# rnaarla/advanced-rag-milvus

Measured on AMD Instinct MI355X. Metric: queries_per_sec_hybrid_retrieve, higher is better.
Workload: dtype f16

## Files before the change

### advanced-rag-milvus_amd/advanced_rag/_native.py

```python
from __future__ import annotations

import ctypes
import os
import threading
from typing import Optional, Sequence, Tuple

import numpy as np

from .staging import csr_of_queries

HR_F32, HR_F16 = 0, 1
HR_METRIC_IP, HR_METRIC_COSINE, HR_METRIC_L2 = 0, 1, 2
HR_METHOD_SEMANTIC, HR_METHOD_SPARSE, HR_METHOD_DOMAIN = 1, 2, 4
HR_MAX_TOPK = 256
HR_NORM_COSINE, HR_NORM_ATAN, HR_NORM_ATAN_DIST, HR_NORM_MINMAX, HR_NORM_MINMAX_DIST = 0, 1, 2, 3, 4
HR_DECAY_GAUSS, HR_DECAY_EXP, HR_DECAY_LINEAR = 0, 1, 2
HR_NORM_NONE = -1
HR_COL_F64 = 5
HR_MAX_DEEP_K = 16384
HR_N_PHASES = 10
PHASE_NAMES = ("prep", "dense_scan", "group_select", "refine", "topk",
               "sparse_scan", "sparse_select", "sparse_refine", "sparse_topk", "finish_fused")
HR_DEBUG_FINISH_MODE, HR_DEBUG_FAIL_NEXT_BUILD, HR_DEBUG_DENSE_KERNELS, HR_DEBUG_SPARSE_RPB, HR_DEBUG_GROUP_ROWS = 1, 2, 3, 4, 5
HR_DEBUG_NO_TRIM = 6
# ... 100 lines not shown
    "hr_decay_rerank_dev": (_c.c_int, [_c.c_void_p, _c.c_void_p, _c.c_int, _c.c_void_p, _c.c_int, _c.c_int, _c.c_void_p, _c.c_int,
                                       _c.c_int64, _c.c_int64, _c.c_void_p, _c.c_int, _c.c_int, _c.c_void_p, _c.c_void_p, _c.c_void_p,
                                       _c.c_void_p, _c.c_void_p]),
    "hr_mask_drop_groups_dev": (_c.c_int, [_c.c_void_p, _c.c_void_p, _c.c_int64, _c.c_void_p, _c.c_void_p, _c.c_int, _c.c_void_p]),
    "hr_group_select_n_dev": (_c.c_int, [_c.c_void_p, _c.c_void_p, _c.c_int, _c.c_int, _c.c_void_p, _c.c_int64, _c.c_int64, _c.c_int,
                                         _c.c_int, _c.c_void_p, _c.c_void_p, _c.c_void_p, _c.c_void_p, _c.c_void_p, _c.c_void_p]),
    "hr_mask_keep_groups_dev": (_c.c_int, [_c.c_void_p, _c.c_void_p, _c.c_int64, _c.c_void_p, _c.c_void_p, _c.c_int, _c.c_void_p]),
    "hr_add_layernorm_f16_dev": (_c.c_int, [_c.c_void_p, _c.c_void_p, _c.c_void_p, _c.c_void_p, _c.c_void_p, _c.c_int64,
                                            _c.c_int, _c.c_float, _c.c_void_p]),
    "hr_embed_layernorm_f16_dev": (_c.c_int, [_c.c_void_p, _c.c_void_p, _c.c_void_p, _c.c_void_p, _c.c_void_p, _c.c_void_p,
                                              _c.c_void_p, _c.c_void_p, _c.c_int64, _c.c_int, _c.c_int, _c.c_float, _c.c_int64,
                                              _c.c_int64, _c.c_void_p]),
    "hr_attention_f16_dev": (_c.c_int, [_c.c_void_p, _c.c_void_p, _c.c_void_p, _c.c_int64, _c.c_int, _c.c_int, _c.c_int,
                                        _c.c_float, _c.c_void_p]),
    "hr_attention_rows_f16_dev": (_c.c_int, [_c.c_void_p, _c.c_int64, _c.c_int64, _c.c_void_p, _c.c_void_p, _c.c_int64, _c.c_int64,
                                             _c.c_void_p, _c.c_void_p, _c.c_int64, _c.c_int, _c.c_int, _c.c_int, _c.c_int, _c.c_float,
                                             _c.c_void_p]),
    "hr_linear_rows_f16_dev": (_c.c_int, [_c.c_void_p, _c.c_int, _c.c_void_p, _c.c_void_p, _c.c_void_p, _c.c_int64, _c.c_int, _c.c_int,
                                          _c.c_int64, _c.c_void_p]),
    "hr_attention_fr_f16_dev": (_c.c_int, [_c.c_void_p, _c.c_void_p, _c.c_void_p, _c.c_int64, _c.c_int, _c.c_int, _c.c_int,
                                           _c.c_float, _c.c_void_p]),
    "hr_encoder_tail_f16_dev": (_c.c_int, [_c.c_void_p, _c.c_void_p, _c.c_int, _c.c_void_p, _c.c_int, _c.c_void_p, _c.c_void_p,
                                           _c.c_int64, _c.c_int, _c.c_int, _c.c_float, _c.c_int, _c.c_void_p]),
    "hr_mask_rows_scratch_bytes": (_c.c_size_t, [_c.c_int64]),
    "hr_mask_rows_dev": (_c.c_int, [_c.c_void_p, _c.c_int64, _c.c_int64, _c.c_int64, _c.c_int64, _c.c_void_p, _c.c_void_p,
                                    _c.c_void_p, _c.c_void_p]),
    "hr_get_dense_rows_dev": (_c.c_int, [_c.c_void_p, _c.c_void_p, _c.c_int64, _c.c_int, _c.c_void_p, _c.c_int64, _c.c_void_p,
                                         _c.c_void_p]),
    "hr_get_dense_rows": (_c.c_int, [_c.c_void_p, _c.c_void_p, _c.c_int64, _c.c_void_p]),
    "hr_get_sparse_rows_scratch_bytes": (_c.c_size_t, [_c.c_int64]),
    "hr_get_sparse_rows_dev": (_c.c_int, [_c.c_void_p, _c.c_void_p, _c.c_int64, _c.c_void_p, _c.c_void_p, _c.c_void_p, _c.c_int64,
                                          _c.c_void_p, _c.c_void_p, _c.c_void_p]),
    "hr_get_sparse_rows": (_c.c_int, [_c.c_void_p, _c.c_void_p, _c.c_int64, _c.c_void_p, _c.c_void_p, _c.c_void_p, _c.c_int64,
                                      _c.c_void_p]),
    "hr_search_dense_deep": (_c.c_int, [_c.c_void_p, _c.c_void_p, _c.c_int, _c.c_int, _c.c_int, _c.c_void_p, _c.c_int, _c.c_void_p,
                                        _c.c_void_p]),
    "hr_search_sparse_deep": (_c.c_int, [_c.c_void_p, _c.c_void_p, _c.c_void_p, _c.c_void_p, _c.c_int, _c.c_int, _c.c_int,
                                         _c.c_float, _c.c_void_p, _c.c_int, _c.c_void_p, _c.c_void_p]),
    "hr_deep_topk_scratch_bytes": (_c.c_size_t, [_c.c_int64, _c.c_int, _c.c_int]),
    "hr_deep_topk_dev": (_c.c_int, [_c.c_void_p, _c.c_void_p, _c.c_int64, _c.c_int, _c.c_int, _c.c_int, _c.c_int, _c.c_int64,
                                    _c.c_void_p, _c.c_void_p, _c.c_void_p, _c.c_void_p]),
    "hr_set_profiling": (_c.c_int, [_c.c_void_p, _c.c_int]),
    "hr_last_kernel_ms": (_c.c_int, [_c.c_void_p, _c.c_void_p, _c.c_int]),
    "hr_last_compact_ms": (_c.c_int, [_c.c_void_p, _c.c_void_p, _c.c_int]),
}
EXPORTED_SYMBOLS = tuple(_SIGNATURES)
# ... 666 lines not shown
    if rc != 0:
        _raise_global(L, rc)


def attention_fr_f16_dev(d_qkv: int, d_lengths: int, d_out_fr: int, n_seq: int, T: int, heads: int, head_dim: int, scale: float,
                         stream: int = 0):
    L = load_library()
    rc = L.hr_attention_fr_f16_dev(_vp(d_qkv), _vp(d_lengths) if d_lengths else None, _vp(d_out_fr), n_seq, T, heads, head_dim,
                                   float(scale), _vp(stream) if stream else None)
    if rc != 0:
        _raise_global(L, rc)


def encoder_tail_f16_dev(d_attn_fr: int, d_x: int, x_fr: bool, d_out: int, out_fr: bool, d_wstream: int, d_tables: int, rows: int,
                         hidden: int, intermediate: int, eps: float, gelu_erf: bool, stream: int = 0):
    L = load_library()
    rc = L.hr_encoder_tail_f16_dev(_vp(d_attn_fr), _vp(d_x), 1 if x_fr else 0, _vp(d_out), 1 if out_fr else 0, _vp(d_wstream),
                                   _vp(d_tables), rows, hidden, intermediate, float(eps), 1 if gelu_erf else 0,
                                   _vp(stream) if stream else None)
    if rc != 0:
        _raise_global(L, rc)


def attention_rows_f16_dev(d_q: int, q_seq_stride: int, q_token_stride: int, d_k: int, d_v: int, kv_seq_stride: int,
                           kv_token_stride: int, d_lengths: int, d_out: int, n_seq: int, T: int, n_queries: int, heads: int,
                           head_dim: int, scale: float, stream: int = 0):
    L = load_library()
    rc = L.hr_attention_rows_f16_dev(_vp(d_q), q_seq_stride, q_token_stride, _vp(d_k), _vp(d_v), kv_seq_stride, kv_token_stride,
                                     _vp(d_lengths) if d_lengths else None, _vp(d_out), n_seq, T, n_queries, heads, head_dim,
                                     float(scale), _vp(stream) if stream else None)
    if rc != 0:
        _raise_global(L, rc)


def rerank_linear_dev(d_ids: int, d_scores: int, d_methods: int, d_n: int, B: int, k_in: int, base_w: float,
                      method_bonus: float, recency_w: float, k_out: int, d_out_ids: int, d_out_scores: int,
                      d_out_orig: int, stream: int = 0, d_recency: int = 0):
    L = load_library()
    rc = L.hr_rerank_linear_dev(_vp(d_ids), _vp(d_scores), _vp(d_methods), _vp(d_n),
                                _vp(d_recency) if d_recency else None, B, k_in, base_w, method_bonus, recency_w,
                                k_out, _vp(d_out_ids), _vp(d_out_scores), _vp(d_out_orig),
                                _vp(stream) if stream else None)
    if rc != 0:
        _raise_global(L, rc)
```

### advanced-rag-milvus_amd/advanced_rag/encoder_kernels.py

```python
from __future__ import annotations

from typing import Optional

import torch

from . import _native

SUPPORTED_TAIL = {(384, 1536)}
SUPPORTED_LINEAR_K = {384}


def pack_natural(w: torch.Tensor) -> torch.Tensor:
    N, K = w.shape
    assert N % 16 == 0 and K % 32 == 0, (N, K)
    v = w.to(torch.float16).reshape(N // 16, 16, K // 32, 4, 8)
    return v.permute(0, 2, 3, 1, 4).contiguous().reshape(-1)


def pack_accumulator_order(w: torch.Tensor) -> torch.Tensor:
    N, K = w.shape
    assert N % 16 == 0 and K % 32 == 0, (N, K)
    v = w.to(torch.float16).reshape(N // 16, 16, K // 32, 2, 4, 4)
    return v.permute(0, 2, 4, 1, 3, 5).contiguous().reshape(-1)

# ... 10 lines not shown
    wp = w[perm]
    return (pack_accumulator_order(wp) if fragment_order_input else pack_natural(wp)), bias[perm].to(torch.float32).contiguous()


def pack_tail_stream(w_out: torch.Tensor, w_up: torch.Tensor, w_down: torch.Tensor) -> torch.Tensor:
    H, I = w_out.shape[0], w_up.shape[0]
    assert w_out.shape == (H, H) and w_up.shape == (I, H) and w_down.shape == (H, I) and H % 32 == 0 and I % 64 == 0
    piece = 512
    sp = H // 16
    out_p = pack_accumulator_order(w_out).reshape(-1, sp * piece)
    up_p = pack_accumulator_order(w_up).reshape(I // 32, sp * piece)
    down_p = pack_accumulator_order(w_down).reshape(H // 16, I // 32, piece).permute(1, 0, 2).reshape(I // 32, sp * piece)
    n = I // 32
    stages = [out_p, up_p[0:1]]
    inter = torch.stack([up_p[1:], down_p[:-1]], dim=1).reshape(2 * (n - 1), sp * piece)
    stages += [inter, down_p[-1:]]
    return torch.cat(stages).reshape(-1).contiguous()


def tail_tables(b_out, g1, be1, b_down, g2, be2, b_up) -> torch.Tensor:
    return torch.cat([t.reshape(-1).to(torch.float32) for t in (b_out, g1, be1, b_down, g2, be2, b_up)]).contiguous()


class LayerKernels:

    def __init__(self):
        self._key = None
        self.qkv_w = self.qkv_w_fr = self.qkv_b = self.kv_w = self.kv_w_fr = self.kv_b = self.stream = self.tables = None

    @staticmethod
    def supports(layer) -> bool:
        H, I = layer.out.weight.shape[0], layer.up.weight.shape[0]
        return (H, I) in SUPPORTED_TAIL and H in SUPPORTED_LINEAR_K

    def ensure(self, layer) -> "LayerKernels":
        params = (layer.qkv.weight, layer.qkv.bias, layer.out.weight, layer.out.bias, layer.ln1.weight, layer.ln1.bias,
                  layer.up.weight, layer.up.bias, layer.down.weight, layer.down.bias, layer.ln2.weight, layer.ln2.bias)
        key = tuple((p.data_ptr(), p._version) for p in params)
        if key != self._key:
            H = layer.out.weight.shape[0]
            with torch.no_grad():
                self.qkv_w, self.qkv_b = pack_linear(layer.qkv.weight, layer.qkv.bias, False)
                self.qkv_w_fr, _ = pack_linear(layer.qkv.weight, layer.qkv.bias, True)
                self.kv_w, self.kv_b = pack_linear(layer.qkv.weight[H:], layer.qkv.bias[H:], False)
                self.kv_w_fr, _ = pack_linear(layer.qkv.weight[H:], layer.qkv.bias[H:], True)
                self.stream = pack_tail_stream(layer.out.weight, layer.up.weight, layer.down.weight)
                self.tables = tail_tables(layer.out.bias, layer.ln1.weight, layer.ln1.bias, layer.down.bias,
                                          layer.ln2.weight, layer.ln2.bias, layer.up.bias)
            self._key = key
        return self


def fr_rows(rows: int) -> int:
    return -(-rows // 16) * 16


def to_fragment_order(x2d: torch.Tensor) -> torch.Tensor:
    M, H = x2d.shape
    pad = torch.zeros((fr_rows(M), H), dtype=x2d.dtype, device=x2d.device)
    pad[:M] = x2d
    v = pad.reshape(-1, 16, H // 32, 2, 4, 4)
    return v.permute(0, 2, 4, 1, 3, 5).contiguous().reshape(fr_rows(M), H)


def from_fragment_order(x_fr: torch.Tensor, rows: int) -> torch.Tensor:
    H = x_fr.shape[1]
    v = x_fr.reshape(-1, H // 32, 4, 16, 2, 4)
    return v.permute(0, 3, 1, 4, 2, 5).contiguous().reshape(-1, H)[:rows]


def linear_rows(x2d: torch.Tensor, w_packed: torch.Tensor, bias_f32: torch.Tensor, n_out: int, rows: Optional[int] = None,
                x_fr: bool = False, out: Optional[torch.Tensor] = None) -> torch.Tensor:
    M = x2d.shape[0] if rows is None else rows
    K = x2d.shape[1]
    if out is None:
        out = torch.empty((M, n_out), dtype=torch.float16, device=x2d.device)
    _native.linear_rows_f16_dev(x2d.data_ptr(), x_fr, w_packed.data_ptr(), bias_f32.data_ptr(), out.data_ptr(), M, K, n_out,
                                out.stride(0), torch.cuda.current_stream(x2d.device).cuda_stream)
    return out


def encoder_tail(attn_fr: torch.Tensor, x2d: torch.Tensor, k: LayerKernels, intermediate: int, eps: float, gelu_erf: bool,
                 rows: Optional[int] = None, x_fr: bool = False, out_fr: bool = False) -> torch.Tensor:
    M = x2d.shape[0] if rows is None else rows
    H = x2d.shape[1]
    out = torch.empty((fr_rows(M) if out_fr else M, H), dtype=torch.float16, device=x2d.device)
    _native.encoder_tail_f16_dev(attn_fr.data_ptr(), x2d.data_ptr(), x_fr, out.data_ptr(), out_fr, k.stream.data_ptr(),
                                 k.tables.data_ptr(), M, H, intermediate, eps, gelu_erf,
                                 torch.cuda.current_stream(x2d.device).cuda_stream)
    return out
```

### advanced-rag-milvus_amd/advanced_rag/encoders.py

```python
from __future__ import annotations

import math
import re
import zlib
from dataclasses import dataclass
from typing import Dict, List, Optional, Sequence, Tuple

import numpy as np
import torch
import torch.nn as nn
import torch.nn.functional as F

from . import _native
from .encoder_kernels import LayerKernels, encoder_tail, fr_rows, linear_rows

_WORD = re.compile(r"\w+|[^\w\s]")
PAD, CLS, SEP = 0, 101, 102


@dataclass
class EncoderConfig:
    vocab_size: int = 30522
    hidden: int = 384
    layers: int = 6
    heads: int = 12
    intermediate: int = 1536
    max_len: int = 512
    type_vocab: int = 2
    eps: float = 1e-12
    gelu: str = "tanh"


class HashTokenizer:

    _MEMO_MAX = 1 << 20

    def __init__(self, vocab_size: int = 30522, max_len: int = 512):
# ... 79 lines not shown

class _Layer(nn.Module):
    def __init__(self, c: EncoderConfig):
        super().__init__()
        self.heads = c.heads
        self.gelu = c.gelu
        self.qkv = nn.Linear(c.hidden, 3 * c.hidden)
        self.out = nn.Linear(c.hidden, c.hidden)
        self.ln1 = nn.LayerNorm(c.hidden, eps=c.eps)
        self.up = nn.Linear(c.hidden, c.intermediate)
        self.down = nn.Linear(c.intermediate, c.hidden)
        self.ln2 = nn.LayerNorm(c.hidden, eps=c.eps)
        self.kernels = LayerKernels()
        self.use_layer_kernels = True

    def _hip_attention_ok(self, x, lengths, hd, T) -> bool:
        return (lengths is not None and x.is_cuda and x.dtype == torch.float16 and
                ((hd == 32 and T <= 1024) or (hd == 64 and T <= 512)))

    def _fused_ok(self, x, lengths, hd, T) -> bool:
        return (self.use_layer_kernels and not getattr(_SMALL, "gemms", False) and self._hip_attention_ok(x, lengths, hd, T)
                and self.gelu in ("tanh", "erf") and LayerKernels.supports(self))

    def forward_fused(self, x2, B, T, lengths, x_fr: bool = False, out_fr: bool = False):
        H = x2.shape[1]
        hd = H // self.heads
        M = B * T
        k = self.kernels.ensure(self)
        if not x2.is_contiguous():
            x2 = x2.contiguous()
        qkv = linear_rows(x2, k.qkv_w_fr if x_fr else k.qkv_w, k.qkv_b, 3 * H, rows=M, x_fr=x_fr)
        a = torch.empty((fr_rows(M), H), dtype=x2.dtype, device=x2.device)
        _native.attention_fr_f16_dev(qkv.data_ptr(), lengths.data_ptr(), a.data_ptr(), B, T, self.heads, hd, hd ** -0.5,
                                     torch.cuda.current_stream(x2.device).cuda_stream)
        return encoder_tail(a, x2, k, self.up.weight.shape[0], float(self.ln1.eps), self.gelu == "erf", rows=M, x_fr=x_fr,
                            out_fr=out_fr)

    def forward(self, x, attn_bias, lengths=None):
        B, T, H = x.shape
        hd = H // self.heads
        if self._fused_ok(x, lengths, hd, T):
            return self.forward_fused(x.reshape(B * T, H), B, T, lengths).view(B, T, H)
        qkv = self.qkv(x)
        if self._hip_attention_ok(x, lengths, hd, T):
            qkv = qkv.contiguous()
            a = torch.empty((B, T, H), dtype=x.dtype, device=x.device)
            _native.attention_f16_dev(qkv.data_ptr(), lengths.data_ptr(), a.data_ptr(), B, T, self.heads, hd, hd ** -0.5,
                                      torch.cuda.current_stream(x.device).cuda_stream)
        else:
            q, k, v = qkv.view(B, T, 3, self.heads, hd).permute(2, 0, 3, 1, 4)
            a = F.scaled_dot_product_attention(q, k, v, attn_mask=attn_bias).transpose(1, 2).reshape(B, T, H)
        x = add_layer_norm(x, self.out(a), self.ln1)
        return add_layer_norm(x, self.down(self._ffn_up(x)), self.ln2)

    def forward_first_token(self, x, mask, lengths=None):
        B, T, H = x.shape
        hd = H // self.heads
        W, b = self.qkv.weight, self.qkv.bias
        if self._fused_ok(x, lengths, hd, T):
            k = self.kernels.ensure(self)
            x2 = x.reshape(B * T, H)
            kv = linear_rows(x2 if x2.is_contiguous() else x2.contiguous(), k.kv_w, k.kv_b, 2 * H).view(B, T, 2 * H)
        else:
            kv = F.linear(x, W[H:], b[H:])
        q = F.linear(x[:, 0], W[:H], b[:H])
        if self._hip_attention_ok(x, lengths, hd, T):
            kv, q = kv.contiguous(), q.contiguous()
            a = torch.empty((B, 1, H), dtype=x.dtype, device=x.device)
            _native.attention_rows_f16_dev(q.data_ptr(), H, 0, kv.data_ptr(), kv.data_ptr() + 2 * H, T * 2 * H, 2 * H,
                                           lengths.data_ptr(), a.data_ptr(), B, T, 1, self.heads, hd, hd ** -0.5,
                                           torch.cuda.current_stream(x.device).cuda_stream)
        else:
            kv = kv.view(B, T, 2, self.heads, hd)
            k, v = kv[:, :, 0].permute(0, 2, 1, 3), kv[:, :, 1].permute(0, 2, 1, 3)
            s = torch.matmul(q.view(B, self.heads, 1, hd), k.transpose(-1, -2)).float() * (hd ** -0.5)
            s = s.masked_fill(~mask[:, None, None, :], float("-inf"))
            a = torch.matmul(torch.softmax(s, dim=-1).to(x.dtype), v).reshape(B, 1, H)
        x0 = add_layer_norm(x[:, :1], self.out(a), self.ln1)
        return add_layer_norm(x0, self.down(self._ffn_up(x0)), self.ln2)

    def _ffn_up(self, x):
        if self.gelu != "tanh":
            return F.gelu(self.up(x))
        if x.is_cuda:
            B, T, H = x.shape
            return torch._addmm_activation(self.up.bias, x.reshape(B * T, H), self.up.weight.t(), use_gelu=True).view(B, T, -1)
        return F.gelu(self.up(x), approximate="tanh")


class BertEncoder(nn.Module):
    def __init__(self, config: Optional[EncoderConfig] = None):
        super().__init__()
        c = self.config = config or EncoderConfig()
        self.word = nn.Embedding(c.vocab_size, c.hidden, padding_idx=PAD)
        self.pos = nn.Embedding(c.max_len, c.hidden)
        self.seg = nn.Embedding(c.type_vocab, c.hidden)
        self.ln = nn.LayerNorm(c.hidden, eps=c.eps)
        self.layers = nn.ModuleList(_Layer(c) for _ in range(c.layers))

    def forward(self, ids, types, mask, first_token_only: bool = False):
        B, T = ids.shape
        if ids.is_cuda and self.word.weight.dtype == torch.float16 and T <= self.pos.weight.shape[0]:
            ids_c, types_c = ids.contiguous().long(), types.contiguous().long()
            H = self.word.weight.shape[1]
            x = torch.empty((B, T, H), dtype=torch.float16, device=ids.device)
            _native.embed_layernorm_f16_dev(ids_c.data_ptr(), types_c.data_ptr(), self.word.weight.data_ptr(),
                                            self.pos.weight.data_ptr(), self.seg.weight.data_ptr(), self.ln.weight.data_ptr(),
                                            self.ln.bias.data_ptr(), x.data_ptr(), B, T, H, float(self.ln.eps),
                                            self.word.weight.shape[0], self.seg.weight.shape[0],
                                            torch.cuda.current_stream(ids.device).cuda_stream)
        else:
            x = add_layer_norm(self.word(ids) + self.pos(torch.arange(T, device=ids.device))[None], self.seg(types), self.ln)
        bias = torch.zeros(mask.shape, dtype=x.dtype, device=x.device).masked_fill(~mask, float("-inf"))[:, None, None, :]
        lengths = mask.sum(dim=1).to(torch.int32) if x.is_cuda and x.dtype == torch.float16 else None
        n_full = len(self.layers) - (1 if first_token_only else 0)
        H = x.shape[-1]
        if n_full and all(layer._fused_ok(x, lengths, H // layer.heads, T) for layer in self.layers[:n_full]):
            x2 = x.reshape(B * T, H)
            for i, layer in enumerate(self.layers[:n_full]):
                x2 = layer.forward_fused(x2, B, T, lengths, x_fr=i > 0, out_fr=i + 1 < n_full)
            x = x2.view(B, T, H)
        else:
            for layer in self.layers[:n_full]:
                x = layer(x, bias, lengths)
        if first_token_only:
            x = self.layers[-1].forward_first_token(x, mask, lengths)
        return x


def _seeded(module_fn, seed: int):
    gen_state = torch.random.get_rng_state()
    torch.manual_seed(seed)
    try:
        m = module_fn()
        for mod in m.modules():
            if isinstance(mod, (nn.Linear, nn.Embedding)):
                nn.init.normal_(mod.weight, std=0.02)
            if isinstance(mod, nn.Linear) and mod.bias is not None:
                nn.init.zeros_(mod.bias)
        return m
    finally:
        torch.random.set_rng_state(gen_state)


_TUNED_GEMMS = None
_SMALL = __import__("threading").local()


def use_recorded_gemm_solutions() -> bool:
# ... 222 lines not shown
```

### advanced-rag-milvus_amd/csrc/encoder_layer.h

```cpp
#pragma once
#include "common.h"

namespace hbmrag {

typedef __attribute__((address_space(1))) const void* el_gptr_t;
typedef __attribute__((address_space(3))) void* el_lptr_t;
typedef _Float16 half4_t __attribute__((ext_vector_type(4)));

#ifndef EL_ABLATE
#define EL_ABLATE 0
#endif
constexpr int kElWaves = 4;
constexpr int kElRingStages = 4;

__device__ inline void el_ds_read4(chunk_t (&a)[4], unsigned addr) {
    asm volatile("ds_read_b128 %0, %4\n\tds_read_b128 %1, %4 offset:1024\n\tds_read_b128 %2, %4 offset:2048\n\tds_read_b128 %3, %4 offset:3072"
                 : "=&v"(a[0]), "=&v"(a[1]), "=&v"(a[2]), "=&v"(a[3]) : "v"(addr) : "memory");
}
template <int N>
__device__ inline void el_wait_lgkm(chunk_t (&a)[4]) {
    asm volatile("s_waitcnt lgkmcnt(%4)" : "+v"(a[0]), "+v"(a[1]), "+v"(a[2]), "+v"(a[3]) : "n"(N) : "memory");
}
__device__ inline f32x4_t el_lds_f4(unsigned addr) {
    f32x4_t v;
// ... 16 lines not shown
__device__ inline void el_load_rows(half8_t (&f)[KS], const _Float16* base, bool fr, bool acc_order, int64_t row0, int64_t M,
                                    int col, int g, int lane) {
    if (fr) {
        const int64_t tile = min(row0, M - 1) >> 4;
        const half8_t* src = reinterpret_cast<const half8_t*>(base) + tile * KS * 64 + lane;
#pragma unroll
        for (int s = 0; s < KS; ++s) f[s] = src[s * 64];
    } else {
        const _Float16* r = base + min(row0 + col, M - 1) * (32 * KS);
        if (acc_order) {
#pragma unroll
            for (int s = 0; s < KS; ++s) {
                const half4_t lo = *reinterpret_cast<const half4_t*>(r + 32 * s + 4 * g);
                const half4_t hi = *reinterpret_cast<const half4_t*>(r + 32 * s + 16 + 4 * g);
                f[s] = (half8_t){lo[0], lo[1], lo[2], lo[3], hi[0], hi[1], hi[2], hi[3]};
            }
        } else {
#pragma unroll
            for (int s = 0; s < KS; ++s) f[s] = *reinterpret_cast<const half8_t*>(r + 32 * s + 8 * g);
        }
    }
}

template <int SP, int NS>
struct ElStream {
    static constexpr int L = SP / kElWaves;
    static_assert(SP % kElWaves == 0 && SP % 4 == 0, "whole pieces per wave, groups of four");
    const chunk_t* stream0;
    const chunk_t* src;
    const chunk_t* src_last;
    chunk_t* ring;
    int issue_slot, read_slot;
    int wid;

    __device__ inline void init(const chunk_t* stream, int64_t n_stages, chunk_t* ring_, int wid_, int lane) {
        stream0 = src = stream + (int64_t)wid_ * kTileChunks + lane;
        src_last = src + (n_stages - 1) * SP * kTileChunks;
        ring = ring_;
        wid = wid_;
        issue_slot = read_slot = 0;
    }
    __device__ inline void issue_piece(int l) {
        if ((EL_ABLATE & 1) && src > stream0 + (int64_t)(NS - 1) * SP * kTileChunks) return;
        const chunk_t* s = src <= src_last ? src : src_last;
        __builtin_amdgcn_global_load_lds((el_gptr_t)(s + l * kElWaves * kTileChunks),
                                         (el_lptr_t)(ring + (issue_slot * SP + wid + l * kElWaves) * kTileChunks), 16, 0, 0);
    }
// ... 108 lines not shown
                half8_t w;
#pragma unroll
                for (int j = 0; j < 8; ++j) w[j] = (_Float16)acc[j >> 2][tt][j & 3];
                *reinterpret_cast<half8_t*>(p.out + row * p.out_stride + 32 * so + 8 * g) = w;
            }
        }
    }
    asm volatile("s_waitcnt vmcnt(0)" ::: "memory");
}

struct TailArgs {
    const _Float16* a;
    const _Float16* x;
    _Float16* out;
    int x_fr, out_fr;
    const chunk_t* wstream;
    const float* tables;
    int64_t M;
    float eps;
#ifdef EL_STAMP
    unsigned long long* stamps;
#endif
};
#ifdef EL_STAMP
#define EL_MARK(i) do { if (threadIdx.x == 0) p.stamps[(size_t)blockIdx.x * 8 + (i)] = __builtin_amdgcn_s_memtime(); } while (0)
#else
#define EL_MARK(i) do { } while (0)
#endif

template <int HS, int IS, int TT, bool ERF>
__global__ __launch_bounds__(64 * kElWaves, 1) void encoder_tail_kernel(TailArgs p) {
    constexpr int H = 32 * HS, I = 32 * IS, HT = 2 * HS, SP = 2 * HS, NS = kElRingStages;
    static_assert(IS % 2 == 0, "the chunk loop is unrolled by two");
    extern __shared__ chunk_t el_lds[];
    const int lane = threadIdx.x & 63;
    const int wid = __builtin_amdgcn_readfirstlane((int)(threadIdx.x >> 6));
    const int col = lane & 15, g = lane >> 4;
    const int64_t tok0 = (int64_t)blockIdx.x * (64 * TT) + wid * (16 * TT);
    float* tbl = reinterpret_cast<float*>(el_lds + NS * SP * kTileChunks);
    const unsigned tbl_lds = (unsigned)(uintptr_t)(el_lptr_t)tbl;
    constexpr unsigned kBout = 0, kG1 = 4u * H, kBe1 = 8u * H, kBdown = 12u * H, kG2 = 16u * H, kBe2 = 20u * H, kBup = 24u * H;

    EL_MARK(0);
    ElStream<SP, NS> st;
    st.init(p.wstream, HS + 2 * IS, el_lds, wid, lane);
#pragma unroll
    for (int s = 0; s < NS - 1; ++s) st.issue();

    for (int i = threadIdx.x; i < (6 * H + I) / 4; i += 64 * kElWaves)
        reinterpret_cast<f32x4_t*>(tbl)[i] = reinterpret_cast<const f32x4_t*>(p.tables)[i];
    half8_t af[TT][HS], res[TT][HS];
#pragma unroll
    for (int tt = 0; tt < TT; ++tt) {
        el_load_rows<HS>(af[tt], p.a, true, true, tok0 + 16 * tt, p.M, col, g, lane);
        el_load_rows<HS>(res[tt], p.x, p.x_fr != 0, true, tok0 + 16 * tt, p.M, col, g, lane);
    }
    __syncthreads();
#pragma unroll
    for (int tt = 0; tt < TT; ++tt)
#pragma unroll
        for (int s = 0; s < HS; ++s) asm volatile("" : "+v"(af[tt][s]), "+v"(res[tt][s]));

    EL_MARK(1);
    f32x4_t o[HT][TT];
#pragma unroll
    for (int so = 0; so < HS; ++so) {
#pragma unroll
        for (int u = 0; u < 2; ++u) {
            const f32x4_t b = el_lds_f4(tbl_lds + kBout + 4u * (16 * (2 * so + u) + 4 * g));
#pragma unroll
            for (int tt = 0; tt < TT; ++tt)
#pragma unroll
// ... 98 lines not shown
    half8_t hfA[TT], hfB[TT];
    auto none = [](int) {};
    up_stage(0, hA, none);
    act_all(hA, hfA, 0);
    act_all(hA, hfA, 1);
    up_stage(1, hB, none);
#pragma unroll 1
    for (int c = 0; c + 2 < IS; c += 2) {
        down_stage(hfA, [&](int gi) { act_part(hB, hfB, 0, gi); });
        up_stage(c + 2, hA, [&](int gi) { act_part(hB, hfB, 1, gi); });
        down_stage(hfB, [&](int gi) { act_part(hA, hfA, 0, gi); });
        up_stage(c + 3, hB, [&](int gi) { act_part(hA, hfA, 1, gi); });
    }
    down_stage(hfA, [&](int gi) { act_part(hB, hfB, 0, gi); });
    act_all(hB, hfB, 1);
    down_stage(hfB, none);

    EL_MARK(4);
    {
        float mean[TT], rstd[TT];
        layer_norm(y, kG2, kBe2, mean, rstd);
    }
    EL_MARK(5);
#pragma unroll
    for (int tt = 0; tt < TT; ++tt) {
        const int64_t row = tok0 + 16 * tt + col;
        if (row < p.M) {
            if (p.out_fr) {
                half8_t* dst = reinterpret_cast<half8_t*>(p.out) + ((tok0 + 16 * tt) >> 4) * HS * 64 + lane;
#pragma unroll
                for (int s = 0; s < HS; ++s) {
                    half8_t w;
#pragma unroll
                    for (int j = 0; j < 8; ++j) w[j] = (_Float16)y[2 * s + (j >> 2)][tt][j & 3];
                    dst[s * 64] = w;
                }
            } else {
#pragma unroll
                for (int t = 0; t < HT; ++t) {
                    half4_t w;
#pragma unroll
                    for (int r = 0; r < 4; ++r) w[r] = (_Float16)y[t][tt][r];
                    *reinterpret_cast<half4_t*>(p.out + row * H + 16 * t + 4 * g) = w;
                }
            }
        }
    }
    asm volatile("s_waitcnt vmcnt(0)" ::: "memory");
    EL_MARK(6);
}

}
```

### advanced-rag-milvus_amd/csrc/hbmrag.hip

```cpp
#include "../../include/hbmrag.h"

#include <hip/hip_runtime.h>

#include <algorithm>
#include <chrono>
#include <cmath>
#include <cstdarg>
#include <cstdio>
#include <cstdlib>
#include <cstring>
#include <map>
#include <mutex>
#include <new>
#include <shared_mutex>
#include <string>
#include <type_traits>
#include <utility>
#include <vector>

#include "common.h"
#include "attention.h"
#include "compact.h"
#include "decay.h"
#include "deep.h"
// ... 2644 lines not shown
    if (rows == 0) return HR_OK;
    constexpr int KS = 12;
    const size_t lds = (size_t)(kElRingStages + 1) * 2 * KS * 1024 + (size_t)N * 4;
    static bool ready = false;
    if (!ready) {
        HR_TRY(el_allow_lds((const void*)linear_rows_kernel<KS, 2>, 160 * 1024));
        HR_TRY(el_allow_lds((const void*)linear_rows_kernel<KS, 4>, 160 * 1024));
        ready = true;
    }
    LinearArgs a{};
    a.x = (const _Float16*)d_x; a.w = (const chunk_t*)d_w_packed; a.bias = d_bias; a.out = (_Float16*)d_out;
    a.M = rows; a.out_stride = out_stride; a.N = N; a.x_fr = x_fr ? 1 : 0;
    const bool wide = rows >= 256 * 256;
    const int rows_per_block = wide ? 256 : 128;
    const int64_t blocks = (rows + rows_per_block - 1) / rows_per_block;
    if (blocks > 0x7fffffffll) return fail(nullptr, HR_ELIMIT, "too many rows");
    if (wide) hipLaunchKernelGGL((linear_rows_kernel<KS, 4>), dim3((unsigned)blocks), dim3(64 * kElWaves), lds, (hipStream_t)stream, a);
    else hipLaunchKernelGGL((linear_rows_kernel<KS, 2>), dim3((unsigned)blocks), dim3(64 * kElWaves), lds, (hipStream_t)stream, a);
    hipError_t e = hipGetLastError();
    if (e != hipSuccess) return fail(nullptr, HR_EHIP, "linear_rows_kernel: %s", hipGetErrorString(e));
    return HR_OK;
}

int hr_encoder_tail_f16_dev(const void* d_attn_fr, const void* d_x, int x_fr, void* d_out, int out_fr, const void* d_wstream,
                            const float* d_tables, int64_t rows, int hidden, int intermediate, float eps, int gelu_erf, void* stream) {
    if (rows < 0 || hidden <= 0 || intermediate <= 0) return fail(nullptr, HR_EINVAL, "bad encoder-tail sizes");
    if (hidden != 384 || intermediate != 1536)
        return fail(nullptr, HR_ELIMIT, "the fused layer tail serves (hidden, intermediate) = (384, 1536) (got %d, %d)", hidden, intermediate);
    if (!d_attn_fr || !d_x || !d_out || !d_wstream || !d_tables) return fail(nullptr, HR_EINVAL, "null buffer");
    if (((uintptr_t)d_attn_fr | (uintptr_t)d_x | (uintptr_t)d_out | (uintptr_t)d_wstream | (uintptr_t)d_tables) & 15)
        return fail(nullptr, HR_EINVAL, "buffers must be 16-byte aligned");
    if (rows == 0) return HR_OK;
    constexpr int HS = 12, IS = 48, TT = 2;
    const size_t lds = (size_t)kElRingStages * 2 * HS * 1024 + (size_t)(6 * hidden + intermediate) * 4;
    static bool ready = false;
    if (!ready) {
        HR_TRY(el_allow_lds((const void*)encoder_tail_kernel<HS, IS, TT, false>, 160 * 1024));
        HR_TRY(el_allow_lds((const void*)encoder_tail_kernel<HS, IS, TT, true>, 160 * 1024));
        ready = true;
    }
    TailArgs a{};
    a.a = (const _Float16*)d_attn_fr; a.x = (const _Float16*)d_x; a.out = (_Float16*)d_out; a.x_fr = x_fr ? 1 : 0; a.out_fr = out_fr ? 1 : 0;
    a.wstream = (const chunk_t*)d_wstream; a.tables = d_tables; a.M = rows; a.eps = eps;
    const int64_t blocks = (rows + 64 * TT - 1) / (64 * TT);
    if (blocks > 0x7fffffffll) return fail(nullptr, HR_ELIMIT, "too many rows");
    if (gelu_erf)
        hipLaunchKernelGGL((encoder_tail_kernel<HS, IS, TT, true>), dim3((unsigned)blocks), dim3(64 * kElWaves), lds, (hipStream_t)stream, a);
    else
        hipLaunchKernelGGL((encoder_tail_kernel<HS, IS, TT, false>), dim3((unsigned)blocks), dim3(64 * kElWaves), lds, (hipStream_t)stream, a);
    hipError_t e = hipGetLastError();
    if (e != hipSuccess) return fail(nullptr, HR_EHIP, "encoder_tail_kernel: %s", hipGetErrorString(e));
    return HR_OK;
}

static int search_dense_host(hr_index* h, const float* q, int B, int k, const uint8_t* rowmask, bool mask_on_device,
                             int64_t* out_ids, float* out_scores, bool ranged = false, const double* radius = nullptr,
                             const double* range_filter = nullptr) {
    HR_TRY(check_search_args(h, B, k, true));
    if (!q || !out_ids || !out_scores) return fail(h, HR_EINVAL, "null buffer");
    for (int64_t i = 0; i < (int64_t)B * h->dim; ++i)
        if (!std::isfinite(q[i])) return fail(h, HR_EINVAL, "non-finite value in query %lld", (long long)(i / h->dim));
    for (int b = 0; ranged && b < B; ++b) {
        const bool l2 = h->metric == HR_METRIC_L2;
        const double r = radius ? radius[b] : (l2 ? INFINITY : -INFINITY);
        const double f = range_filter ? range_filter[b] : (l2 ? -INFINITY : INFINITY);
        if (std::isnan(r) || std::isnan(f)) return fail(h, HR_EINVAL, "NaN range bound in query %d", b);
        if (l2 ? f >= r : r >= f)
            return fail(h, HR_EINVAL, "empty range in query %d: radius %g, range_filter %g (%s)", b, r, f,
                        l2 ? "L2 keeps range_filter <= distance < radius" : "kept are radius < score <= range_filter");
    }
    DenseRange rng{nullptr, nullptr};
    return search_host(
        h, B, k, &hr_index::n_rows, rowmask, mask_on_device, out_ids, out_scores,
        [&](Workspace* ws, hipStream_t s) {
            HIP_TRY(h, ws->d_q.ensure((size_t)B * h->dim * 4));
// ... 475 lines not shown
```

### include/hbmrag.h

```cpp
#ifndef HBMRAG_H
#define HBMRAG_H

#include <stdint.h>
#include <stddef.h>

#if defined(HR_BUILD)
#define HR_API __attribute__((visibility("default")))
#else
#define HR_API
#endif

#ifdef __cplusplus
extern "C" {
#endif

typedef struct hr_index hr_index;

typedef enum hr_status {
    HR_OK = 0,
    HR_EINVAL = 1,
    HR_ESTATE = 2,
    HR_EHIP = 3,
    HR_ENOMEM = 4,
    HR_ELIMIT = 5
// ... 215 lines not shown
HR_API int hr_hash_tokenize_dev(const uint8_t* d_text, const int64_t* d_off, int n, int max_len, int vocab, int64_t* d_ids,
                         int32_t* d_lens, int32_t* d_flags, void* stream);

HR_API int hr_add_layernorm_f16_dev(const void* d_x, const void* d_residual, const void* d_gamma, const void* d_beta,
                             void* d_out, int64_t rows, int hidden, float eps, void* stream);

HR_API int hr_embed_layernorm_f16_dev(const int64_t* d_ids, const int64_t* d_types, const void* d_word, const void* d_pos,
                               const void* d_seg, const void* d_gamma, const void* d_beta, void* d_out, int64_t n_seq, int T,
                               int hidden, float eps, int64_t n_word, int64_t n_seg, void* stream);

HR_API int hr_attention_f16_dev(const void* d_qkv, const int32_t* d_lengths, void* d_out, int64_t n_seq, int T, int heads,
                         int head_dim, float scale, void* stream);
HR_API int hr_attention_rows_f16_dev(const void* d_q, int64_t q_seq_stride, int64_t q_token_stride, const void* d_k, const void* d_v,
                              int64_t kv_seq_stride, int64_t kv_token_stride, const int32_t* d_lengths, void* d_out,
                              int64_t n_seq, int T, int n_queries, int heads, int head_dim, float scale, void* stream);

HR_API int hr_linear_rows_f16_dev(const void* d_x, int x_fr, const void* d_w_packed, const float* d_bias, void* d_out, int64_t rows,
                           int K, int N, int64_t out_stride, void* stream);
HR_API int hr_attention_fr_f16_dev(const void* d_qkv, const int32_t* d_lengths, void* d_out_fr, int64_t n_seq, int T, int heads,
                            int head_dim, float scale, void* stream);
HR_API int hr_encoder_tail_f16_dev(const void* d_attn_fr, const void* d_x, int x_fr, void* d_out, int out_fr, const void* d_wstream,
                            const float* d_tables, int64_t rows, int hidden, int intermediate, float eps, int gelu_erf,
                            void* stream);

HR_API int hr_stream_create(int device, int priority, const uint32_t* cu_mask, int n_words, void** out_stream);
HR_API int hr_stream_destroy(int device, void* stream);
HR_API int hr_set_scan_cus(hr_index* h, int n_cus);

enum { HR_DEBUG_FINISH_MODE = 1, HR_DEBUG_FAIL_NEXT_BUILD = 2, HR_DEBUG_DENSE_KERNELS = 3, HR_DEBUG_SPARSE_RPB = 4,
       HR_DEBUG_GROUP_ROWS = 5, HR_DEBUG_NO_TRIM = 6, HR_DEBUG_NO_RANGE_CLAMP = 7 };
HR_API int hr_debug_option(hr_index* h, int key, int value);

#define HR_N_PHASES 10
HR_API int hr_set_profiling(hr_index* h, int enabled);
HR_API int hr_last_kernel_ms(hr_index* h, float* out_ms, int n);
HR_API int hr_last_compact_ms(hr_index* h, float* out_ms, int n);
HR_API int64_t hr_dense_scan_bytes(const hr_index* h);

#ifdef __cplusplus
}
#endif
#endif
```

Baseline: 32770.

## Fuse next layer's QKV/KV projection into the encoder tail kernel

Extends the fused encoder-tail kernel so that after the second layernorm it immediately multiplies the output rows by the next layer's QKV (or KV-only for the first-token last layer) weights, streamed through the same LDS ring. This removes a separate linear_rows launch per layer and the re-read of the hidden state from memory. For the last full layer it writes only every T-th row of the hidden output, since only the first token is needed. It adds extra weight-stream length and LDS table space per block, plus register pressure from the held half-precision copies of the output rows.

Result: no change. 32730 (-0.1%).

```diff
diff --git a/advanced-rag-milvus_amd/advanced_rag/_native.py b/advanced-rag-milvus_amd/advanced_rag/_native.py
--- a/advanced-rag-milvus_amd/advanced_rag/_native.py
+++ b/advanced-rag-milvus_amd/advanced_rag/_native.py
@@ -146,6 +146,9 @@
                                            _c.c_float, _c.c_void_p]),
     "hr_encoder_tail_f16_dev": (_c.c_int, [_c.c_void_p, _c.c_void_p, _c.c_int, _c.c_void_p, _c.c_int, _c.c_void_p, _c.c_void_p,
                                            _c.c_int64, _c.c_int, _c.c_int, _c.c_float, _c.c_int, _c.c_void_p]),
+    "hr_encoder_tail_next_f16_dev": (_c.c_int, [_c.c_void_p, _c.c_void_p, _c.c_int, _c.c_void_p, _c.c_int, _c.c_int64, _c.c_void_p,
+                                                _c.c_void_p, _c.c_void_p, _c.c_int64, _c.c_int, _c.c_int64, _c.c_int, _c.c_int,
+                                                _c.c_float, _c.c_int, _c.c_void_p]),
     "hr_mask_rows_scratch_bytes": (_c.c_size_t, [_c.c_int64]),
     "hr_mask_rows_dev": (_c.c_int, [_c.c_void_p, _c.c_int64, _c.c_int64, _c.c_int64, _c.c_int64, _c.c_void_p, _c.c_void_p,
                                     _c.c_void_p, _c.c_void_p]),
@@ -858,6 +861,17 @@
         _raise_global(L, rc)
 
 
+def encoder_tail_next_f16_dev(d_attn_fr: int, d_x: int, x_fr: bool, d_out: int, out_fr: bool, out_every: int, d_wstream: int,
+                              d_tables: int, d_next_out: int, next_stride: int, next_n: int, rows: int, hidden: int,
+                              intermediate: int, eps: float, gelu_erf: bool, stream: int = 0):
+    L = load_library()
+    rc = L.hr_encoder_tail_next_f16_dev(_vp(d_attn_fr), _vp(d_x), 1 if x_fr else 0, _vp(d_out), 1 if out_fr else 0, out_every,
+                                        _vp(d_wstream), _vp(d_tables), _vp(d_next_out), next_stride, next_n, rows, hidden,
+                                        intermediate, float(eps), 1 if gelu_erf else 0, _vp(stream) if stream else None)
+    if rc != 0:
+        _raise_global(L, rc)
+
+
 def attention_rows_f16_dev(d_q: int, q_seq_stride: int, q_token_stride: int, d_k: int, d_v: int, kv_seq_stride: int,
                            kv_token_stride: int, d_lengths: int, d_out: int, n_seq: int, T: int, n_queries: int, heads: int,
                            head_dim: int, scale: float, stream: int = 0):
diff --git a/advanced-rag-milvus_amd/advanced_rag/encoder_kernels.py b/advanced-rag-milvus_amd/advanced_rag/encoder_kernels.py
--- a/advanced-rag-milvus_amd/advanced_rag/encoder_kernels.py
+++ b/advanced-rag-milvus_amd/advanced_rag/encoder_kernels.py
@@ -56,11 +56,20 @@
     return torch.cat([t.reshape(-1).to(torch.float32) for t in (b_out, g1, be1, b_down, g2, be2, b_up)]).contiguous()
 
 
+def extend_tail_stream(stream: torch.Tensor, w_next_fr: torch.Tensor) -> torch.Tensor:
+    return torch.cat([stream.reshape(-1), w_next_fr.reshape(-1)]).contiguous()
+
+
+def extend_tail_tables(tables: torch.Tensor, b_next: torch.Tensor) -> torch.Tensor:
+    return torch.cat([tables, b_next.reshape(-1).to(torch.float32)]).contiguous()
+
+
 class LayerKernels:
 
     def __init__(self):
         self._key = None
         self.qkv_w = self.qkv_w_fr = self.qkv_b = self.kv_w = self.kv_w_fr = self.kv_b = self.stream = self.tables = None
+        self._next = {}
 
     @staticmethod
     def supports(layer) -> bool:
@@ -82,7 +91,18 @@
                 self.tables = tail_tables(layer.out.bias, layer.ln1.weight, layer.ln1.bias, layer.down.bias,
                                           layer.ln2.weight, layer.ln2.bias, layer.up.bias)
             self._key = key
+            self._next = {}
         return self
+
+    def ensure_next(self, layer, next_layer, kv_only: bool):
+        self.ensure(layer)
+        nk = next_layer.kernels.ensure(next_layer)
+        key = (self._key, nk._key)
+        hit = self._next.get(kv_only)
+        if hit is None or hit[0] != key:
+            w, b = (nk.kv_w_fr, nk.kv_b) if kv_only else (nk.qkv_w_fr, nk.qkv_b)
+            hit = self._next[kv_only] = (key, extend_tail_stream(self.stream, w), extend_tail_tables(self.tables, b))
+        return hit[1], hit[2]
 
 
 def fr_rows(rows: int) -> int:
@@ -123,3 +143,19 @@
                                  k.tables.data_ptr(), M, H, intermediate, eps, gelu_erf,
                                  torch.cuda.current_stream(x2d.device).cuda_stream)
     return out
+
+
+def encoder_tail_next(attn_fr: torch.Tensor, x2d: torch.Tensor, stream_next: torch.Tensor, tables_next: torch.Tensor,
+                      next_n: int, intermediate: int, eps: float, gelu_erf: bool, rows: Optional[int] = None,
+                      x_fr: bool = False, out_fr: bool = False, out_every: int = 0, out: Optional[torch.Tensor] = None,
+                      next_out: Optional[torch.Tensor] = None):
+    M = x2d.shape[0] if rows is None else rows
+    H = x2d.shape[1]
+    if out is None:
+        out = torch.empty((fr_rows(M) if out_fr else M, H), dtype=torch.float16, device=x2d.device)
+    if next_out is None:
+        next_out = torch.empty((M, next_n), dtype=torch.float16, device=x2d.device)
+    _native.encoder_tail_next_f16_dev(attn_fr.data_ptr(), x2d.data_ptr(), x_fr, out.data_ptr(), out_fr, out_every,
+                                      stream_next.data_ptr(), tables_next.data_ptr(), next_out.data_ptr(), next_out.stride(0),
+                                      next_n, M, H, intermediate, eps, gelu_erf, torch.cuda.current_stream(x2d.device).cuda_stream)
+    return out, next_out
diff --git a/advanced-rag-milvus_amd/advanced_rag/encoders.py b/advanced-rag-milvus_amd/advanced_rag/encoders.py
--- a/advanced-rag-milvus_amd/advanced_rag/encoders.py
+++ b/advanced-rag-milvus_amd/advanced_rag/encoders.py
@@ -12,7 +12,7 @@
 import torch.nn.functional as F
 
 from . import _native
-from .encoder_kernels import LayerKernels, encoder_tail, fr_rows, linear_rows
+from .encoder_kernels import LayerKernels, encoder_tail, encoder_tail_next, fr_rows, linear_rows
 
 _WORD = re.compile(r"\w+|[^\w\s]")
 PAD, CLS, SEP = 0, 101, 102
@@ -138,17 +138,24 @@
         return (self.use_layer_kernels and not getattr(_SMALL, "gemms", False) and self._hip_attention_ok(x, lengths, hd, T)
                 and self.gelu in ("tanh", "erf") and LayerKernels.supports(self))
 
-    def forward_fused(self, x2, B, T, lengths, x_fr: bool = False, out_fr: bool = False):
+    def forward_fused(self, x2, B, T, lengths, x_fr: bool = False, out_fr: bool = False, qkv=None, next_layer=None,
+                      next_first_token: bool = False):
         H = x2.shape[1]
         hd = H // self.heads
         M = B * T
         k = self.kernels.ensure(self)
         if not x2.is_contiguous():
             x2 = x2.contiguous()
-        qkv = linear_rows(x2, k.qkv_w_fr if x_fr else k.qkv_w, k.qkv_b, 3 * H, rows=M, x_fr=x_fr)
+        if qkv is None:
+            qkv = linear_rows(x2, k.qkv_w_fr if x_fr else k.qkv_w, k.qkv_b, 3 * H, rows=M, x_fr=x_fr)
         a = torch.empty((fr_rows(M), H), dtype=x2.dtype, device=x2.device)
         _native.attention_fr_f16_dev(qkv.data_ptr(), lengths.data_ptr(), a.data_ptr(), B, T, self.heads, hd, hd ** -0.5,
                                      torch.cuda.current_stream(x2.device).cuda_stream)
+        if next_layer is not None:
+            stream, tables = k.ensure_next(self, next_layer, next_first_token)
+            return encoder_tail_next(a, x2, stream, tables, (2 if next_first_token else 3) * H, self.up.weight.shape[0],
+                                     float(self.ln1.eps), self.gelu == "erf", rows=M, x_fr=x_fr, out_fr=out_fr,
+                                     out_every=T if next_first_token else 0)
         return encoder_tail(a, x2, k, self.up.weight.shape[0], float(self.ln1.eps), self.gelu == "erf", rows=M, x_fr=x_fr,
                             out_fr=out_fr)
 
@@ -169,11 +176,13 @@
         x = add_layer_norm(x, self.out(a), self.ln1)
         return add_layer_norm(x, self.down(self._ffn_up(x)), self.ln2)
 
-    def forward_first_token(self, x, mask, lengths=None):
+    def forward_first_token(self, x, mask, lengths=None, kv=None):
         B, T, H = x.shape
         hd = H // self.heads
         W, b = self.qkv.weight, self.qkv.bias
-        if self._fused_ok(x, lengths, hd, T):
+        if kv is not None:
+            kv = kv.view(B, T, 2 * H)
+        elif self._fused_ok(x, lengths, hd, T):
             k = self.kernels.ensure(self)
             x2 = x.reshape(B * T, H)
             kv = linear_rows(x2 if x2.is_contiguous() else x2.contiguous(), k.kv_w, k.kv_b, 2 * H).view(B, T, 2 * H)
@@ -213,6 +222,7 @@
         self.seg = nn.Embedding(c.type_vocab, c.hidden)
         self.ln = nn.LayerNorm(c.hidden, eps=c.eps)
         self.layers = nn.ModuleList(_Layer(c) for _ in range(c.layers))
+        self.fuse_next_projection = True
 
     def forward(self, ids, types, mask, first_token_only: bool = False):
         B, T = ids.shape
@@ -231,16 +241,23 @@
         lengths = mask.sum(dim=1).to(torch.int32) if x.is_cuda and x.dtype == torch.float16 else None
         n_full = len(self.layers) - (1 if first_token_only else 0)
         H = x.shape[-1]
+        kv = None
         if n_full and all(layer._fused_ok(x, lengths, H // layer.heads, T) for layer in self.layers[:n_full]):
-            x2 = x.reshape(B * T, H)
+            x2, qkv = x.reshape(B * T, H), None
             for i, layer in enumerate(self.layers[:n_full]):
-                x2 = layer.forward_fused(x2, B, T, lengths, x_fr=i > 0, out_fr=i + 1 < n_full)
-            x = x2.view(B, T, H)
+                last_full = i + 1 == n_full
+                nxt = self.layers[i + 1] if self.fuse_next_projection and (not last_full or first_token_only) else None
+                if last_full and nxt is not None and not nxt._fused_ok(x, lengths, H // nxt.heads, T):
+                    nxt = None
+                out = layer.forward_fused(x2, B, T, lengths, x_fr=i > 0, out_fr=not last_full, qkv=qkv, next_layer=nxt,
+                                          next_first_token=last_full)
+                x2, qkv = out if nxt is not None else (out, None)
+            x, kv = x2.view(B, T, H), qkv
         else:
             for layer in self.layers[:n_full]:
                 x = layer(x, bias, lengths)
         if first_token_only:
-            x = self.layers[-1].forward_first_token(x, mask, lengths)
+            x = self.layers[-1].forward_first_token(x, mask, lengths, kv=kv)
         return x
 
 
diff --git a/advanced-rag-milvus_amd/csrc/encoder_layer.h b/advanced-rag-milvus_amd/csrc/encoder_layer.h
--- a/advanced-rag-milvus_amd/csrc/encoder_layer.h
+++ b/advanced-rag-milvus_amd/csrc/encoder_layer.h
@@ -62,7 +62,7 @@
     }
 }
 
-template <int SP, int NS>
+template <int SP, int NS, int KERNEL = 0>
 struct ElStream {
     static constexpr int L = SP / kElWaves;
     static_assert(SP % kElWaves == 0 && SP % 4 == 0, "whole pieces per wave, groups of four");
@@ -217,14 +217,20 @@
     unsigned long long* stamps;
 #endif
 };
+struct TailNextArgs : TailArgs {
+    int next_N;
+    _Float16* next_out;
+    int64_t next_stride;
+    int64_t out_every;
+};
 #ifdef EL_STAMP
 #define EL_MARK(i) do { if (threadIdx.x == 0) p.stamps[(size_t)blockIdx.x * 8 + (i)] = __builtin_amdgcn_s_memtime(); } while (0)
 #else
 #define EL_MARK(i) do { } while (0)
 #endif
 
-template <int HS, int IS, int TT, bool ERF>
-__global__ __launch_bounds__(64 * kElWaves, 1) void encoder_tail_kernel(TailArgs p) {
+template <int HS, int IS, int TT, bool ERF, int NEXT = 0>
+__global__ __launch_bounds__(64 * kElWaves, 1) void encoder_tail_kernel(std::conditional_t<NEXT != 0, TailNextArgs, TailArgs> p) {
     constexpr int H = 32 * HS, I = 32 * IS, HT = 2 * HS, SP = 2 * HS, NS = kElRingStages;
     static_assert(IS % 2 == 0, "the chunk loop is unrolled by two");
     extern __shared__ chunk_t el_lds[];
@@ -235,14 +241,17 @@
     float* tbl = reinterpret_cast<float*>(el_lds + NS * SP * kTileChunks);
     const unsigned tbl_lds = (unsigned)(uintptr_t)(el_lptr_t)tbl;
     constexpr unsigned kBout = 0, kG1 = 4u * H, kBe1 = 8u * H, kBdown = 12u * H, kG2 = 16u * H, kBe2 = 20u * H, kBup = 24u * H;
+    constexpr unsigned kBnext = 4u * (6 * H + I);
+    int n_next = 0;
+    if constexpr (NEXT) n_next = p.next_N / 32;
 
     EL_MARK(0);
-    ElStream<SP, NS> st;
-    st.init(p.wstream, HS + 2 * IS, el_lds, wid, lane);
+    ElStream<SP, NS, NEXT> st;
+    st.init(p.wstream, HS + 2 * IS + n_next, el_lds, wid, lane);
 #pragma unroll
     for (int s = 0; s < NS - 1; ++s) st.issue();
 
-    for (int i = threadIdx.x; i < (6 * H + I) / 4; i += 64 * kElWaves)
+    for (int i = threadIdx.x; i < (6 * H + I) / 4 + 8 * n_next; i += 64 * kElWaves)
         reinterpret_cast<f32x4_t*>(tbl)[i] = reinterpret_cast<const f32x4_t*>(p.tables)[i];
     half8_t af[TT][HS], res[TT][HS];
 #pragma unroll
@@ -387,26 +396,83 @@
         layer_norm(y, kG2, kBe2, mean, rstd);
     }
     EL_MARK(5);
-#pragma unroll
-    for (int tt = 0; tt < TT; ++tt) {
-        const int64_t row = tok0 + 16 * tt + col;
-        if (row < p.M) {
-            if (p.out_fr) {
-                half8_t* dst = reinterpret_cast<half8_t*>(p.out) + ((tok0 + 16 * tt) >> 4) * HS * 64 + lane;
-#pragma unroll
-                for (int s = 0; s < HS; ++s) {
+    if constexpr (NEXT) {
+        half8_t yf[TT][HS];
+#pragma unroll
+        for (int tt = 0; tt < TT; ++tt)
+#pragma unroll
+            for (int s = 0; s < HS; ++s)
+#pragma unroll
+                for (int j = 0; j < 8; ++j) yf[tt][s][j] = (_Float16)y[2 * s + (j >> 2)][tt][j & 3];
+#pragma unroll
+        for (int tt = 0; tt < TT; ++tt) {
+            const int64_t row = tok0 + 16 * tt + col;
+            if (row < p.M && (p.out_every == 0 || row % p.out_every == 0)) {
+                if (p.out_fr) {
+                    half8_t* dst = reinterpret_cast<half8_t*>(p.out) + ((tok0 + 16 * tt) >> 4) * HS * 64 + lane;
+#pragma unroll
+                    for (int s = 0; s < HS; ++s) dst[s * 64] = yf[tt][s];
+                } else {
+#pragma unroll
+                    for (int s = 0; s < HS; ++s)
+#pragma unroll
+                        for (int u = 0; u < 2; ++u) {
+                            half4_t w;
+#pragma unroll
+                            for (int r = 0; r < 4; ++r) w[r] = yf[tt][s][4 * u + r];
+                            *reinterpret_cast<half4_t*>(p.out + row * H + 16 * (2 * s + u) + 4 * g) = w;
+                        }
+                }
+            }
+        }
+#pragma unroll 1
+        for (int so = 0; so < n_next; ++so) {
+            f32x4_t acc[2][TT];
+#pragma unroll
+            for (int u = 0; u < 2; ++u) {
+                const f32x4_t b = el_lds_f4(tbl_lds + kBnext + 4u * (32 * so + 16 * u + 4 * g));
+#pragma unroll
+                for (int tt = 0; tt < TT; ++tt) acc[u][tt] = b;
+            }
+            const unsigned addr = st.begin(lane);
+            st.consume(addr, [&](int pi, half8_t a) {
+                const int u = pi / HS, s = pi % HS;
+#pragma unroll
+                for (int tt = 0; tt < TT; ++tt) acc[u][tt] = __builtin_amdgcn_mfma_f32_16x16x32_f16(a, yf[tt][s], acc[u][tt], 0, 0, 0);
+            });
+#pragma unroll
+            for (int tt = 0; tt < TT; ++tt) {
+                const int64_t row = tok0 + 16 * tt + col;
+                if (row < p.M) {
                     half8_t w;
 #pragma unroll
-                    for (int j = 0; j < 8; ++j) w[j] = (_Float16)y[2 * s + (j >> 2)][tt][j & 3];
-                    dst[s * 64] = w;
+                    for (int j = 0; j < 8; ++j) w[j] = (_Float16)acc[j >> 2][tt][j & 3];
+                    *reinterpret_cast<half8_t*>(p.next_out + row * p.next_stride + 32 * so + 8 * g) = w;
                 }
-            } else {
-#pragma unroll
-                for (int t = 0; t < HT; ++t) {
-                    half4_t w;
-#pragma unroll
-                    for (int r = 0; r < 4; ++r) w[r] = (_Float16)y[t][tt][r];
-                    *reinterpret_cast<half4_t*>(p.out + row * H + 16 * t + 4 * g) = w;
+            }
+        }
+    } else {
+#pragma unroll
+        for (int tt = 0; tt < TT; ++tt) {
+            const int64_t row = tok0 + 16 * tt + col;
+            if (row < p.M) {
+                if (p.out_fr) {
+                    half8_t* dst = reinterpret_cast<half8_t*>(p.out) + ((tok0 + 16 * tt) >> 4) * HS * 64 + lane;
+#pragma unroll
+                    for (int s = 0; s < HS; ++s) {
+                        half8_t w;
+#pragma unroll
+                        for (int j = 0; j < 8; ++j) w[j] = (_Float16)y[2 * s + (j >> 2)][tt][j & 3];
+                        dst[s * 64] = w;
+                    }
+                } else {
+#pragma unroll
+                    for (int t = 0; t < HT; ++t) {
+                        half4_t w;
+#pragma unroll
+                        for (int r = 0; r < 4; ++r) w[r] = (_Float16)y[t][tt][r];
+                        *reinterpret_cast<half4_t*>(p.out + row * H + 16 * t + 4 * g) = w;
+                    }
                 }
             }
         }
diff --git a/advanced-rag-milvus_amd/csrc/hbmrag.hip b/advanced-rag-milvus_amd/csrc/hbmrag.hip
--- a/advanced-rag-milvus_amd/csrc/hbmrag.hip
+++ b/advanced-rag-milvus_amd/csrc/hbmrag.hip
@@ -2690,35 +2690,62 @@
     return HR_OK;
 }
 
-int hr_encoder_tail_f16_dev(const void* d_attn_fr, const void* d_x, int x_fr, void* d_out, int out_fr, const void* d_wstream,
-                            const float* d_tables, int64_t rows, int hidden, int intermediate, float eps, int gelu_erf, void* stream) {
+static int encoder_tail_launch(const void* d_attn_fr, const void* d_x, int x_fr, void* d_out, int out_fr, int64_t out_every,
+                               const void* d_wstream, const float* d_tables, void* d_next_out, int64_t next_stride, int next_N,
+                               int64_t rows, int hidden, int intermediate, float eps, int gelu_erf, void* stream) {
     if (rows < 0 || hidden <= 0 || intermediate <= 0) return fail(nullptr, HR_EINVAL, "bad encoder-tail sizes");
     if (hidden != 384 || intermediate != 1536)
         return fail(nullptr, HR_ELIMIT, "the fused layer tail serves (hidden, intermediate) = (384, 1536) (got %d, %d)", hidden, intermediate);
     if (!d_attn_fr || !d_x || !d_out || !d_wstream || !d_tables) return fail(nullptr, HR_EINVAL, "null buffer");
     if (((uintptr_t)d_attn_fr | (uintptr_t)d_x | (uintptr_t)d_out | (uintptr_t)d_wstream | (uintptr_t)d_tables) & 15)
         return fail(nullptr, HR_EINVAL, "buffers must be 16-byte aligned");
+    const bool next = next_N != 0;
+    if (next) {
+        if (next_N < 0 || next_N % 32 != 0 || next_stride < next_N || next_stride % 8 != 0 || out_every < 0)
+            return fail(nullptr, HR_EINVAL, "bad next-projection sizes");
+        if (next_N > 4096) return fail(nullptr, HR_ELIMIT, "N exceeds 4096");
+        if (!d_next_out) return fail(nullptr, HR_EINVAL, "null buffer");
+        if ((uintptr_t)d_next_out & 15) return fail(nullptr, HR_EINVAL, "buffers must be 16-byte aligned");
+    }
     if (rows == 0) return HR_OK;
     constexpr int HS = 12, IS = 48, TT = 2;
-    const size_t lds = (size_t)kElRingStages * 2 * HS * 1024 + (size_t)(6 * hidden + intermediate) * 4;
+    const size_t lds = (size_t)kElRingStages * 2 * HS * 1024 + (size_t)(6 * hidden + intermediate + next_N) * 4;
     static bool ready = false;
     if (!ready) {
         HR_TRY(el_allow_lds((const void*)encoder_tail_kernel<HS, IS, TT, false>, 160 * 1024));
         HR_TRY(el_allow_lds((const void*)encoder_tail_kernel<HS, IS, TT, true>, 160 * 1024));
+        HR_TRY(el_allow_lds((const void*)encoder_tail_kernel<HS, IS, TT, false, 1>, 160 * 1024));
+        HR_TRY(el_allow_lds((const void*)encoder_tail_kernel<HS, IS, TT, true, 1>, 160 * 1024));
         ready = true;
     }
-    TailArgs a{};
+    TailNextArgs a{};
     a.a = (const _Float16*)d_attn_fr; a.x = (const _Float16*)d_x; a.out = (_Float16*)d_out; a.x_fr = x_fr ? 1 : 0; a.out_fr = out_fr ? 1 : 0;
     a.wstream = (const chunk_t*)d_wstream; a.tables = d_tables; a.M = rows; a.eps = eps;
+    a.next_N = next_N; a.next_out = (_Float16*)d_next_out; a.next_stride = next_stride; a.out_every = out_every;
     const int64_t blocks = (rows + 64 * TT - 1) / (64 * TT);
     if (blocks > 0x7fffffffll) return fail(nullptr, HR_ELIMIT, "too many rows");
-    if (gelu_erf)
-        hipLaunchKernelGGL((encoder_tail_kernel<HS, IS, TT, true>), dim3((unsigned)blocks), dim3(64 * kElWaves), lds, (hipStream_t)stream, a);
-    else
-        hipLaunchKernelGGL((encoder_tail_kernel<HS, IS, TT, false>), dim3((unsigned)blocks), dim3(64 * kElWaves), lds, (hipStream_t)stream, a);
+    const dim3 grid((unsigned)blocks), block(64 * kElWaves);
+    if (next && gelu_erf) hipLaunchKernelGGL((encoder_tail_kernel<HS, IS, TT, true, 1>), grid, block, lds, (hipStream_t)stream, a);
+    else if (next) hipLaunchKernelGGL((encoder_tail_kernel<HS, IS, TT, false, 1>), grid, block, lds, (hipStream_t)stream, a);
+    else if (gelu_erf) hipLaunchKernelGGL((encoder_tail_kernel<HS, IS, TT, true>), grid, block, lds, (hipStream_t)stream, (TailArgs)a);
+    else hipLaunchKernelGGL((encoder_tail_kernel<HS, IS, TT, false>), grid, block, lds, (hipStream_t)stream, (TailArgs)a);
     hipError_t e = hipGetLastError();
     if (e != hipSuccess) return fail(nullptr, HR_EHIP, "encoder_tail_kernel: %s", hipGetErrorString(e));
     return HR_OK;
+}
+
+int hr_encoder_tail_f16_dev(const void* d_attn_fr, const void* d_x, int x_fr, void* d_out, int out_fr, const void* d_wstream,
+                            const float* d_tables, int64_t rows, int hidden, int intermediate, float eps, int gelu_erf, void* stream) {
+    return encoder_tail_launch(d_attn_fr, d_x, x_fr, d_out, out_fr, 0, d_wstream, d_tables, nullptr, 0, 0, rows, hidden, intermediate,
+                               eps, gelu_erf, stream);
+}
+
+int hr_encoder_tail_next_f16_dev(const void* d_attn_fr, const void* d_x, int x_fr, void* d_out, int out_fr, int64_t out_every,
+                                 const void* d_wstream, const float* d_tables, void* d_next_out, int64_t next_stride, int next_N,
+                                 int64_t rows, int hidden, int intermediate, float eps, int gelu_erf, void* stream) {
+    if (next_N <= 0) return fail(nullptr, HR_EINVAL, "bad next-projection sizes");
+    return encoder_tail_launch(d_attn_fr, d_x, x_fr, d_out, out_fr, out_every, d_wstream, d_tables, d_next_out, next_stride, next_N,
+                               rows, hidden, intermediate, eps, gelu_erf, stream);
 }
 
 static int search_dense_host(hr_index* h, const float* q, int B, int k, const uint8_t* rowmask, bool mask_on_device,
diff --git a/include/hbmrag.h b/include/hbmrag.h
--- a/include/hbmrag.h
+++ b/include/hbmrag.h
@@ -261,6 +261,9 @@
 HR_API int hr_encoder_tail_f16_dev(const void* d_attn_fr, const void* d_x, int x_fr, void* d_out, int out_fr, const void* d_wstream,
                             const float* d_tables, int64_t rows, int hidden, int intermediate, float eps, int gelu_erf,
                             void* stream);
+HR_API int hr_encoder_tail_next_f16_dev(const void* d_attn_fr, const void* d_x, int x_fr, void* d_out, int out_fr, int64_t out_every,
+                                 const void* d_wstream, const float* d_tables, void* d_next_out, int64_t next_stride, int next_N,
+                                 int64_t rows, int hidden, int intermediate, float eps, int gelu_erf, void* stream);
 
 HR_API int hr_stream_create(int device, int priority, const uint32_t* cu_mask, int n_words, void** out_stream);
 HR_API int hr_stream_destroy(int device, void* stream);
```
